# yxlao/deepSpeech

Hardware: AMD Instinct MI355X
Metric: audio-sec/sec training throughput (whole node), DS2 BiGRU (higher is better)
Workload: dtype bf16; 1 GPU; model=DeepSpeech2 2xconv(32) + 5xBiGRU-800 bidirectional + CTC, global_batch=32, seq_len=1000, parallelism=dp1, engine=hip

## Files before the change

deepspeech_amd/csrc/api.h:

```cpp
#pragma once
#include <hip/hip_runtime_api.h>
#include <stddef.h>

extern "C" {

struct DS2Fill {
  int n;
  unsigned* ptr[8];
  unsigned long long words[8];
  unsigned pattern[8];
};

hipEvent_t ds2_take_stop_event();
void ds2_arm_stop_event(hipEvent_t e);

int ds2_multi_fill(int n, void* const* ptrs, const unsigned long long* bytes, const unsigned* patterns,
                   hipStream_t st);
int ds2_multi_copy(int n, void* const* dst, const void* const* src, const unsigned long long* rows,
                   const unsigned* src_row, const unsigned* dst_row, const unsigned* src_pitch,
                   const unsigned* dst_pitch, float* sdst, const float* svals, int ns, hipStream_t st);
int ds2_wait_resident(const unsigned* word, long long timeout, hipStream_t st);
int ds2_prep_inputs(const float* x, void* y, long long n, const int* lens_in, int* lens_out, int nl,
                    hipStream_t st);
int ds2_transpose_bf16(const void* in, void* out, int R, int C, int ldi, int ldo, hipStream_t st);
// ... 214 lines not shown
                      int F, int nF, int nT, int inplace, hipStream_t st);

int ds2_seq_dropout(const void* x, void* out, const int* ctr, int T, int N, int H, unsigned seed_lo,
                    unsigned seed_hi, int site, int thr, float scale, int locked, hipStream_t st);

struct DS2Conv1WgradBn {
  const void *dz, *y1;
  const float *mean, *invstd, *gamma, *beta, *dbeta, *dgamma;
};

struct DS2Conv2DgradBn {
  const void* y1;
  const float *mean, *invstd, *gamma, *beta;
  float* part;
};

const char* ds2_conv_status_str(int rc);
size_t ds2_conv2_fwd_smem(int F1);
size_t ds2_conv2_dgrad_smem(int F2);
size_t ds2_conv2_wgrad_smem(int F1);
long long ds2_conv2_wgrad_part_floats(int grid);
long long ds2_conv1_wgrad_part_floats(int grid);
int ds2_conv1_fwd_grid(int N, int T1);
int ds2_conv1_fwd(const void* x, const void* w, const float* bias, void* y, float* part, int N, int T, int F0,
                  int T1, int F1, hipStream_t st);
int ds2_conv2_fwd(const void* x, const void* w, const float* bias, void* y, float* part, int grid, int N, int T1,
                  int F1, int T2, int F2, long long* trace, hipStream_t st);
int ds2_conv2_dgrad(const void* dy, const void* w, void* dx, int grid, int N, int T1, int F1, int T2, int F2,
                    const DS2Conv2DgradBn* bn, long long* trace, hipStream_t st);
int ds2_conv2_wgrad(const void* dy, const void* x, float* part, int grid, float* dw, int N, int T1, int F1, int T2,
                    int F2, hipStream_t st);
int ds2_conv1_wgrad(const void* dy, const void* x, float* part, int grid, float* dw, int N, int T, int F0, int T1,
                    int F1, const DS2Conv1WgradBn* bn, hipStream_t st);
int ds2_bn_cl_finalize(const float* part, int nb, double M, float eps, float* mean, float* invstd, float* run_mean,
                       float* run_var, float momentum, hipStream_t st);
int ds2_bn_cl_apply(const void* y, const float* mean, const float* invstd, const float* gamma, const float* beta,
                    void* out, int N, int T, int F, int tmaj, hipStream_t st);
int ds2_bn_cl_bwd(const void* dz, const void* y, const float* mean, const float* invstd, const float* gamma,
                  const float* beta, float* part, int nb, float* dgamma, float* dbeta, void* dy, int N, int T, int F,
                  int tmaj, int part_ready, hipStream_t st);

struct DS2Feat {
  const void* pcm;
  long long row_stride;
  int S, lead, mode, B, T_max;
  const int* lens;
  const float* offset;
  const float* gain;
  const float* basis;
  const int* mel_idx;
  const float* mel_w;
  const float* dct;
  const float* lifter;
  void* out;
  int* frames;
};

int ds2_audio_stats(const void* pcm, int in_i16, long long row_stride, int S, int B, const int* lens, float* offset,
                    float* gain, hipStream_t st);
int ds2_featurize(const DS2Feat* a, int kind, int in_i16, int out_bf16, hipStream_t st);

int ds2_resample_tile();
int ds2_resample_supported(int L, int M, int K);
int ds2_resample(const void* x, int in_i16, long long row_stride, int S, int B, const int* lens, const float* h,
                 int L, int M, int K, int in_off, int ph0, int n_out, int to_end, float* out, int* out_lens,
                 hipStream_t st);
// ... 3 lines not shown
```

deepspeech_amd/csrc/bindings.cpp:

```cpp
#include <torch/extension.h>
#include <c10/hip/HIPStream.h>
#include <hip/hip_runtime.h>

#include <algorithm>
#include <cstdint>
#include <string>
#include <utility>
#include <vector>

#include "api.h"

namespace {

using OptT = c10::optional<at::Tensor>;

hipStream_t cur_stream() { return c10::hip::getCurrentHIPStream().stream(); }

void check(int rc, const char* what) {
  TORCH_CHECK(rc == 0, "deepspeech_amd kernel launch failed in ", what, " (code ", rc, ")");
}
void check_conv(int rc, const char* what) {
  const char* why = ds2_conv_status_str(rc);
  TORCH_CHECK(rc == 0, "deepspeech_amd kernel launch failed in ", what, " (code ", rc, ")", why ? ": " : "",
              why ? why : "");
// ... 557 lines not shown
  need_bf16(x, "x"); need_bf16(w, "w"); need_bf16(y, "y");
  TORCH_CHECK(x.dim() == 4 && y.dim() == 4 && x.size(3) == 32 && y.size(3) == 32 && w.numel() == 32 * 32 * 50,
              "conv2_fwd shapes");
  TORCH_CHECK(grid > 0, "grid");
  need_f32(part, "part", grid * 64);
  check_conv(ds2_conv2_fwd(x.data_ptr(), w.data_ptr(), ptr_or_null<float>(bias, "bias"), y.data_ptr(),
                           part.data_ptr<float>(), (int)grid, (int)x.size(0), (int)x.size(1), (int)x.size(2),
                           (int)y.size(1), (int)y.size(2), trace_ptr(trace), cur_stream()), "conv2_fwd");
}

void conv2_dgrad(at::Tensor dy, at::Tensor w, at::Tensor dx, int64_t grid, OptT y1, OptT mean, OptT invstd,
                 OptT gamma, OptT beta, OptT part, OptT trace) {
  need_bf16(dy, "dy"); need_bf16(w, "w"); need_bf16(dx, "dx");
  TORCH_CHECK(dy.dim() == 4 && dx.dim() == 4 && dy.size(3) == 32 && dx.size(3) == 32 && w.numel() == 32 * 32 * 50,
              "conv2_dgrad shapes");
  TORCH_CHECK(grid > 0, "grid");
  DS2Conv2DgradBn bn{};
  const bool with_bn = y1.has_value();
  if (with_bn) {
    TORCH_CHECK(mean && invstd && gamma && beta && part, "conv2_dgrad: the BN arguments come all or none");
    need_bf16(*y1, "y1");
    TORCH_CHECK(y1->sizes() == dx.sizes(), "y1 must have dx's shape");
    need_f32(*mean, "mean", 32); need_f32(*invstd, "invstd", 32); need_f32(*gamma, "gamma", 32);
    need_f32(*beta, "beta", 32); need_f32(*part, "part", grid * 64);
    bn = DS2Conv2DgradBn{y1->data_ptr(), mean->data_ptr<float>(), invstd->data_ptr<float>(),
                         gamma->data_ptr<float>(), beta->data_ptr<float>(), part->data_ptr<float>()};
  }
  check_conv(ds2_conv2_dgrad(dy.data_ptr(), w.data_ptr(), dx.data_ptr(), (int)grid, (int)dx.size(0), (int)dx.size(1),
                             (int)dx.size(2), (int)dy.size(1), (int)dy.size(2), with_bn ? &bn : nullptr,
                             trace_ptr(trace), cur_stream()),
             "conv2_dgrad");
}

void conv2_wgrad(at::Tensor dy, at::Tensor x, at::Tensor part, at::Tensor dw, int64_t grid) {
  need_bf16(dy, "dy"); need_bf16(x, "x");
  TORCH_CHECK(grid > 0, "grid");
  need_f32(part, "part", ds2_conv2_wgrad_part_floats((int)grid));
  need_f32(dw, "dw", 32 * 32 * 50);
  check_conv(ds2_conv2_wgrad(dy.data_ptr(), x.data_ptr(), part.data_ptr<float>(), (int)grid, dw.data_ptr<float>(),
                             (int)x.size(0), (int)x.size(1), (int)x.size(2), (int)dy.size(1), (int)dy.size(2),
                             cur_stream()), "conv2_wgrad");
}

void conv1_wgrad(at::Tensor dy, at::Tensor x, at::Tensor part, at::Tensor dw, int64_t grid, OptT y1, OptT mean,
                 OptT invstd, OptT gamma, OptT beta, OptT dbeta, OptT dgamma) {
  need_bf16(dy, "dy"); need_bf16(x, "x");
  TORCH_CHECK(grid > 0, "grid");
  need_f32(part, "part", ds2_conv1_wgrad_part_floats((int)grid));
  need_f32(dw, "dw", 32 * 100);
  DS2Conv1WgradBn bn{};
  const bool with_bn = y1.has_value();
  if (with_bn) {
    TORCH_CHECK(mean && invstd && gamma && beta && dbeta && dgamma, "conv1_wgrad: the BN arguments come all or none");
    need_bf16(*y1, "y1");
    TORCH_CHECK(y1->sizes() == dy.sizes(), "y1 must have dz's shape");
    for (const OptT* t : {&mean, &invstd, &gamma, &beta, &dbeta, &dgamma}) need_f32(**t, "bn vector", 32);
    bn = DS2Conv1WgradBn{dy.data_ptr(), y1->data_ptr(), mean->data_ptr<float>(), invstd->data_ptr<float>(),
                         gamma->data_ptr<float>(), beta->data_ptr<float>(), dbeta->data_ptr<float>(),
                         dgamma->data_ptr<float>()};
  }
  check_conv(ds2_conv1_wgrad(with_bn ? nullptr : dy.data_ptr(), x.data_ptr(), part.data_ptr<float>(), (int)grid,
                             dw.data_ptr<float>(), (int)x.size(0), (int)x.size(1), (int)x.size(2), (int)dy.size(1),
                             (int)dy.size(2), with_bn ? &bn : nullptr, cur_stream()), "conv1_wgrad");
}
int64_t conv2_wgrad_part_floats(int64_t grid) { return ds2_conv2_wgrad_part_floats((int)grid); }
int64_t conv1_wgrad_part_floats(int64_t grid) { return ds2_conv1_wgrad_part_floats((int)grid); }

void bn_cl_finalize(at::Tensor part, int64_t nb, double M, double eps, at::Tensor mean, at::Tensor invstd,
                    OptT run_mean, OptT run_var, double momentum) {
  need_f32(part, "part", nb * 64);
  need_f32(mean, "mean", 32); need_f32(invstd, "invstd", 32);
  check_conv(ds2_bn_cl_finalize(part.data_ptr<float>(), (int)nb, M, (float)eps, mean.data_ptr<float>(),
                                invstd.data_ptr<float>(), ptr_or_null<float>(run_mean, "run_mean"),
                                ptr_or_null<float>(run_var, "run_var"), (float)momentum, cur_stream()),
             "bn_cl_finalize");
}

void bn_cl_apply(at::Tensor y, at::Tensor mean, at::Tensor invstd, at::Tensor gamma, at::Tensor beta, at::Tensor out,
                 bool tmaj) {
  need_bf16(y, "y"); need_bf16(out, "out");
  TORCH_CHECK(y.dim() == 4 && y.size(3) == 32 && out.numel() == y.numel(), "bn_cl_apply shapes");
  need_f32(mean, "mean", 32); need_f32(invstd, "invstd", 32); need_f32(gamma, "gamma", 32); need_f32(beta, "beta", 32);
  check_conv(ds2_bn_cl_apply(y.data_ptr(), mean.data_ptr<float>(), invstd.data_ptr<float>(), gamma.data_ptr<float>(),
                             beta.data_ptr<float>(), out.data_ptr(), (int)y.size(0), (int)y.size(1), (int)y.size(2),
                             tmaj ? 1 : 0, cur_stream()), "bn_cl_apply");
}

void bn_cl_bwd(at::Tensor dz, at::Tensor y, at::Tensor mean, at::Tensor invstd, at::Tensor gamma, at::Tensor beta,
               at::Tensor part, int64_t nb, at::Tensor dgamma, at::Tensor dbeta, at::Tensor dy, bool tmaj,
               int64_t part_ready) {
  need_bf16(dz, "dz"); need_bf16(y, "y"); need_bf16(dy, "dy");
  TORCH_CHECK(y.dim() == 4 && y.size(3) == 32 && dz.numel() == y.numel() && dy.numel() == y.numel(),
              "bn_cl_bwd shapes");
  need_f32(part, "part", nb * 64);
  need_f32(mean, "mean", 32); need_f32(invstd, "invstd", 32); need_f32(gamma, "gamma", 32); need_f32(beta, "beta", 32);
  need_f32(dgamma, "dgamma", 32); need_f32(dbeta, "dbeta", 32);
// ... 888 lines not shown
        py::arg("a_col"), py::arg("b_col"), py::arg("ws"), py::arg("cnt"), py::arg("max_grid"));
  m.def("gemm8_splits", [](int64_t K, bool fp8, int64_t S) { return ds2_gemm8_splits((int)K, fp8 ? 1 : 0, (int)S); });
  m.def("multi_fill", &multi_fill);
  m.def("col_sum", &col_sum);
  m.def("wait_resident", &wait_resident);
  m.def("fc_bias_grad", &fc_bias_grad);
  m.def("ctc_beam", &ctc_beam);
  m.def("ctc_beam_backtrack", &ctc_beam_backtrack);
  m.def("ctc_beam_lm", &ctc_beam_lm);
  m.def("ctc_beam_backtrack_lm", &ctc_beam_backtrack_lm);
  m.def("event_new", &event_new, py::arg("flags") = 0);
  m.def("arm_stop_event", &arm_stop_event);
  m.def("disarm_stop_event", &disarm_stop_event);
  m.def("event_free", &event_free);
  m.def("event_record", &event_record);
  m.def("event_wait", &event_wait);
  m.def("event_query", &event_query);
  m.def("stream_wait", &stream_wait);
  m.def("ctc_greedy", &ctc_greedy, py::arg("logits"), py::arg("lens"), py::arg("labels"), py::arg("counts"),
        py::arg("blank"), py::arg("score") = py::none());
  m.def("conv1_fwd", &conv1_fwd);
  m.def("conv1_fwd_grid", &conv1_fwd_grid);
  m.def("conv2_fwd", &conv2_fwd, py::arg("x"), py::arg("w"), py::arg("bias"), py::arg("y"), py::arg("part"),
        py::arg("grid"), py::arg("trace") = py::none());
  m.def("conv2_dgrad", &conv2_dgrad, py::arg("dy"), py::arg("w"), py::arg("dx"), py::arg("grid"),
        py::arg("y1") = py::none(), py::arg("mean") = py::none(), py::arg("invstd") = py::none(),
        py::arg("gamma") = py::none(), py::arg("beta") = py::none(), py::arg("part") = py::none(),
        py::arg("trace") = py::none());
  m.def("conv2_wgrad", &conv2_wgrad);
  m.def("conv1_wgrad", &conv1_wgrad, py::arg("dy"), py::arg("x"), py::arg("part"), py::arg("dw"), py::arg("grid"),
        py::arg("y1") = py::none(), py::arg("mean") = py::none(), py::arg("invstd") = py::none(),
        py::arg("gamma") = py::none(), py::arg("beta") = py::none(), py::arg("dbeta") = py::none(),
        py::arg("dgamma") = py::none());
  m.def("conv2_wgrad_part_floats", &conv2_wgrad_part_floats);
  m.def("conv1_wgrad_part_floats", &conv1_wgrad_part_floats);
  m.def("bn_cl_finalize", &bn_cl_finalize);
  m.def("bn_cl_apply", &bn_cl_apply);
  m.def("bn_cl_bwd", &bn_cl_bwd, py::arg("dz"), py::arg("y"), py::arg("mean"), py::arg("invstd"), py::arg("gamma"),
        py::arg("beta"), py::arg("part"), py::arg("nb"), py::arg("dgamma"), py::arg("dbeta"), py::arg("dy"),
        py::arg("tmaj"), py::arg("part_ready") = 0);
  m.def("gemm", &gemm, py::arg("A"), py::arg("B"), py::arg("C"), py::arg("bias"), py::arg("M"), py::arg("N"),
        py::arg("K"), py::arg("a_col"), py::arg("b_col"), py::arg("epi"), py::arg("alpha"), py::arg("cfg"),
        py::arg("alpha_dev") = py::none(), py::arg("Ml") = 0, py::arg("Nl") = 0, py::arg("Kl") = 0,
        py::arg("fill") = std::vector<at::Tensor>{}, py::arg("fill_pat") = std::vector<int64_t>{});
  m.def("gemm_tile", &gemm_tile);
  m.def("head_ctc", &head_ctc, py::arg("h"), py::arg("W"), py::arg("bias"), py::arg("lens"), py::arg("labels"),
        py::arg("label_lens"), py::arg("loss"), py::arg("G"), py::arg("ws"), py::arg("blank"), py::arg("zero_inf"),
        py::arg("mean") = py::none(), py::arg("counter") = py::none(), py::arg("first_bad") = py::none());
  m.def("fc_logits", &fc_logits);
  m.def("lookahead", &lookahead);
  m.def("lookahead_wgrad_parts", &lookahead_wgrad_parts);
  m.def("lookahead_wgrad", &lookahead_wgrad);
  m.def("lookahead_stream", &lookahead_stream);
  m.def("specaug_plan", &specaug_plan);
  m.def("specaug_mean", &specaug_mean);
  m.def("specaug_apply", &specaug_apply, py::arg("x"), py::arg("lens"), py::arg("plan"), py::arg("fill"),
        py::arg("out"), py::arg("nF"), py::arg("nT"), py::arg("inplace"));
  m.def("seq_dropout", &seq_dropout, py::arg("x"), py::arg("out"), py::arg("ctr"), py::arg("seed_lo"),
        py::arg("seed_hi"), py::arg("site"), py::arg("thr"), py::arg("scale"), py::arg("locked"));
  m.def("audio_stats", &audio_stats, py::arg("pcm"), py::arg("lens"), py::arg("offset"), py::arg("gain"));
  m.def("featurize", &featurize, py::arg("pcm"), py::arg("lens"), py::arg("offset"), py::arg("gain"),
        py::arg("basis"), py::arg("mel_idx"), py::arg("mel_w"), py::arg("dct"), py::arg("lifter"), py::arg("kind"),
        py::arg("lead"), py::arg("mode"), py::arg("out"), py::arg("frames"));
  m.def("resample", &resample, py::arg("pcm"), py::arg("lens"), py::arg("h"), py::arg("L"), py::arg("M"),
        py::arg("in_off"), py::arg("ph0"), py::arg("to_end"), py::arg("out"), py::arg("out_lens"));
  m.def("resample_tile", []() { return ds2_resample_tile(); });
// ... 15 lines not shown
```

deepspeech_amd/csrc/conv1.hip:

```cpp
#include "bn_math.h"
#include "conv_common.h"

using namespace ds2;

namespace {

struct Conv1Fwd {
  const bf16_t* x;
  const bf16_t* w;
  const float* bias;
  bf16_t* y;
  float* part;
  int N, T, F0, T1, F1;
};
constexpr int C1_KT = 20, C1_KF = 5;
constexpr int C1_XS = 200;
constexpr int C1_ROWS = 4;
constexpr int C1_IN = 2 * (C1_ROWS - 1) + C1_KT;

__device__ __forceinline__ void stage_rows(bf16_t* xs, const bf16_t* xu, int t0, int T, int F0) {
  constexpr int NE = C1_IN * C1_XS, K = (NE + 255) / 256;
  bf16_t v[K];
#pragma unroll
  for (int k = 0; k < K; ++k) {
    const int idx = min((int)threadIdx.x + 256 * k, NE - 1);
    const int r = idx / C1_XS, c = idx - r * C1_XS;
    v[k] = xu[(size_t)min(t0 + r, T - 1) * F0 + min(c, F0 - 1)];
  }
#pragma unroll
  for (int k = 0; k < K; ++k) {
    const int idx = (int)threadIdx.x + 256 * k;
    const int r = idx / C1_XS, c = idx - r * C1_XS;
    if (idx < NE) xs[idx] = (t0 + r < T && c < F0) ? v[k] : (bf16_t)0;
  }
}

__global__ __launch_bounds__(256) void conv1_fwd_kernel(Conv1Fwd a) {
  __shared__ __attribute__((aligned(16))) bf16_t xs[C1_IN * C1_XS];
  __shared__ __attribute__((aligned(16))) bf16_t ys[C1_ROWS][32 * MT * CC];
  __shared__ float statsh[4 * 32 * 2];
  const int tid = threadIdx.x, lane = tid & 63, w = uni(tid >> 6);
  const int hi = lane >> 5, col = lane & 31;
  const int tb = (a.T1 + C1_ROWS - 1) / C1_ROWS;
  const int n = blockIdx.x / tb, t1_0 = (blockIdx.x - n * tb) * C1_ROWS;
  stage_rows(xs, a.x + (size_t)n * a.T * a.F0, 2 * t1_0, a.T, a.F0);
  bf16x8 bfr[10];
#pragma unroll
  for (int s = 0; s < 10; ++s) {
    const int kt = 2 * s + hi;
    bf16x8 v;
#pragma unroll
    for (int j = 0; j < 8; ++j) v[j] = j < C1_KF ? (short)a.w[(col * C1_KT + kt) * C1_KF + j] : (short)0;
    bfr[s] = v;
  }
  const float bco = a.bias ? a.bias[col] : 0.f;
  __syncthreads();
  float ssum = 0.f, ssq = 0.f;
  const int t1 = t1_0 + w;
  if (t1 < a.T1) {
    f32x16 acc[MT];
#pragma unroll
    for (int m = 0; m < MT; ++m) acc[m] = (f32x16){};
#pragma unroll
    for (int s = 0; s < 10; ++s) {
      const int r = 2 * w + 2 * s + hi;
#pragma unroll
      for (int m = 0; m < MT; ++m) {
// ... 3 lines not shown
        acc[m] = mfma32(av, bfr[s], acc[m]);
      }
    }
    bf16_t* yl = ys[w];
#pragma unroll
    for (int m = 0; m < MT; ++m)
#pragma unroll
      for (int r = 0; r < 16; ++r) {
        const int f1 = 32 * m + (r & 3) + 8 * (r >> 2) + 4 * hi;
        if (f1 < a.F1) {
          const bf16_t b = f2bf(acc[m][r] + bco);
          yl[f1 * CC + col] = b;
          const float vb = bf2f(b);
          ssum += vb;
          ssq += vb * vb;
        }
      }
    copy_row(a.y + ((size_t)n * a.T1 + t1) * a.F1 * CC, yl, a.F1 * 4, lane, 64);
  }
  channel_sums(ssum, ssq, statsh, w, a.part);
}

struct Conv1Wgrad {
  const bf16_t* dy;
  const bf16_t* x;
  float* part;
  int N, T, F0, T1, F1;
  DS2Conv1WgradBn bn;
  float M;
};
constexpr int C1W_XP = 88;
constexpr int C1W_DY = C1_ROWS * 80 * 64;
constexpr int C1W_XD = C1_IN * 8 * C1W_XP * 2;
constexpr int C1W_RED = 4 * 5 * 4 * 64 * 16;
constexpr int C1W_RAW = C1_IN * C1_XS * 2;
constexpr int C1W_SMEM = (C1W_DY + C1W_XD + C1W_RAW) > C1W_RED ? (C1W_DY + C1W_XD + C1W_RAW) : C1W_RED;

__global__ __launch_bounds__(256) void conv1_wgrad_kernel(Conv1Wgrad a) {
  extern __shared__ __attribute__((aligned(16))) unsigned char smem[];
  const int tid = threadIdx.x, lane = tid & 63, w = uni(tid >> 6);
  const int hi = lane >> 5, col = lane & 31;
  unsigned char* dys = smem;
  bf16_t* xd = (bf16_t*)(smem + C1W_DY);
  bf16_t* raw = (bf16_t*)(smem + C1W_DY + C1W_XD);
  const int tb = (a.T1 + C1_ROWS - 1) / C1_ROWS;
  const int ntiles = a.N * tb;
  const unsigned lofs = tr_lane_ofs(lane);
  const int bkt = col >> 3, bkf = col & 7;

  const bool bn = a.bn.dz != nullptr;
  const bf16_t *bdz = (const bf16_t*)a.bn.dz, *by1 = (const bf16_t*)a.bn.y1;
  float bmu[8], bis[8], bg[8], bbt[8], bmdb[8], bmdg[8];
  if (bn) {
#pragma unroll
    for (int j = 0; j < 8; ++j) {
      const int c = (tid & 3) * 8 + j;
      bmu[j] = a.bn.mean[c]; bis[j] = a.bn.invstd[c]; bg[j] = a.bn.gamma[c]; bbt[j] = a.bn.beta[c];
      bmdb[j] = a.bn.dbeta[c] / a.M; bmdg[j] = a.bn.dgamma[c] / a.M;
    }
  }
  f32x16 acc[5];
#pragma unroll
  for (int i = 0; i < 5; ++i) acc[i] = (f32x16){};
  for (int tile = blockIdx.x; tile < ntiles; tile += gridDim.x) {
    const int n = tile / tb, t1_0 = (tile - n * tb) * C1_ROWS;
    __syncthreads();
    for (int ch = tid; ch < C1_ROWS * 80 * 4; ch += 256) {
      const int r = ch / 320, rem = ch - r * 320, pos = rem >> 2, c4 = rem & 3;
      const int t1 = t1_0 + r;
      i32x4 v = (i32x4){0, 0, 0, 0};
      if (pos < a.F1 && t1 < a.T1) {
        const size_t off = (((size_t)n * a.T1 + t1) * a.F1 + pos) * CC + c4 * 8;
        if (bn) {
          const bf16x8 y = *(const bf16x8*)(by1 + off), d = *(const bf16x8*)(bdz + off);
          bf16x8 o;
#pragma unroll
          for (int j = 0; j < 8; ++j) {
            const float xh = bn_xhat(bf2f((bf16_t)y[j]), bmu[j], bis[j]);
            const float dd = bn_masked(xh, bg[j], bbt[j], bf2f((bf16_t)d[j]));
            o[j] = (short)f2bf(bn_bwd_value(bg[j] * bis[j], dd, xh, bmdb[j], bmdg[j]));
          }
          v = __builtin_bit_cast(i32x4, o);
        } else {
          v = *(const i32x4*)(a.dy + off);
        }
      }
      *(i32x4*)(dys + ch * 16) = v;
    }
    stage_rows(raw, a.x + (size_t)n * a.T * a.F0, 2 * t1_0, a.T, a.F0);
    __syncthreads();
    for (int ch = tid; ch < C1_IN * 8 * 10; ch += 256) {
      const int kf = ch & 7, q = ch >> 3, r = q / 10, p0 = (q - r * 10) * 8;
      bf16x8 v;
#pragma unroll
      for (int j = 0; j < 8; ++j) v[j] = (short)raw[r * C1_XS + min(2 * (p0 + j) + kf, C1_XS - 1)];
      *(bf16x8*)(xd + (r * 8 + kf) * C1W_XP + p0) = v;
    }
    __syncthreads();
    const int t1 = t1_0 + w;
    if (t1 < a.T1) {
#pragma unroll
      for (int kk = 0; kk < 5; ++kk) {
        const unsigned k0 = (unsigned)(16 * kk);
        const bf16x8 av = tr_frag(dys + (w * 80 + k0) * 64 + lofs);
#pragma unroll
        for (int nt = 0; nt < 5; ++nt) {
          const int r = 2 * w + 4 * nt + bkt;
          const bf16x8 bv = *(const bf16x8*)(xd + (r * 8 + bkf) * C1W_XP + k0 + 8 * hi);
          acc[nt] = mfma32(av, bv, acc[nt]);
        }
      }
    }
  }
  __syncthreads();
  f32x4* red = (f32x4*)smem;
#pragma unroll
  for (int nt = 0; nt < 5; ++nt)
#pragma unroll
    for (int r4 = 0; r4 < 4; ++r4) red[((w * 5 + nt) * 4 + r4) * 64 + lane] = acc4(acc[nt], r4);
  __syncthreads();
  f32x4* out = (f32x4*)(a.part + (size_t)blockIdx.x * 5 * 1024);
  for (int e = tid; e < 5 * 4 * 64; e += 256) {
    f32x4 v = red[e];
    for (int wv = 1; wv < 4; ++wv) v += red[wv * 5 * 4 * 64 + e];
    out[e] = v;
  }
}

bool conv1_geometry(int T, int F0, int T1, int F1, int F1max) {
  return F1 <= F1max && F1 == (F0 - 5) / 2 + 1 && T1 == (T - 20) / 2 + 1 && T1 >= 1;
}

}

extern "C" {

long long ds2_conv1_wgrad_part_floats(int grid) { return (long long)grid * 5 * 1024; }
int ds2_conv1_fwd_grid(int N, int T1) { return N * ((T1 + C1_ROWS - 1) / C1_ROWS); }

int ds2_conv1_fwd(const void* x, const void* w, const float* bias, void* y, float* part, int N, int T, int F0,
                  int T1, int F1, hipStream_t st) {
  if (!conv1_geometry(T, F0, T1, F1, 96)) return CONV1_FWD_GEOMETRY;
  Conv1Fwd a{(const bf16_t*)x, (const bf16_t*)w, bias, (bf16_t*)y, part, N, T, F0, T1, F1};
  hipLaunchKernelGGL(conv1_fwd_kernel, dim3(ds2_conv1_fwd_grid(N, T1)), dim3(256), 0, st, a);
  return (int)hipGetLastError();
}

int ds2_conv1_wgrad(const void* dy, const void* x, float* part, int grid, float* dw, int N, int T, int F0, int T1,
                    int F1, const DS2Conv1WgradBn* bn, hipStream_t st) {
  if (!conv1_geometry(T, F0, T1, F1, 80)) return CONV1_WGRAD_GEOMETRY;
  if ((dy == nullptr) == (bn == nullptr)) return CONV1_WGRAD_DY_XOR_BN;
  DS2_HIP_CHECK((hipError_t)set_smem(conv1_wgrad_kernel, C1W_SMEM));
  Conv1Wgrad a{(const bf16_t*)dy, (const bf16_t*)x, part, N, T, F0, T1, F1, bn ? *bn : DS2Conv1WgradBn{},
               (float)((double)N * T1 * F1)};
  hipLaunchKernelGGL(conv1_wgrad_kernel, dim3(grid), dim3(256), C1W_SMEM, st, a);
  hipLaunchKernelGGL(wgrad_reduce_kernel<1>, dim3(5 * 1024 / 256), dim3(256), 0, st, part, grid, 5 * 1024, dw);
  return (int)hipGetLastError();
}

}
```

deepspeech_amd/csrc/conv2.hip:

```cpp
#include "bn_math.h"
#include "conv_common.h"

using namespace ds2;

namespace {

constexpr int PR = 80;

template <int KPW, int S0, typename Idx>
__device__ __forceinline__ void gather_wfrag(bf16x8 (&bfr)[KPW], const unsigned short* wl, int hh, int hi, int col,
                                             Idx idx) {
#pragma unroll
  for (int i = 0; i < KPW; ++i) {
    const int s = S0 + i;
    if ((s & 1) != hh) continue;
    const int kt = s / 10, kf = (s % 10) >> 1;
#pragma unroll
    for (int j = 0; j < 8; ++j) bfr[i][j] = (short)wl[idx(8 * hi + j, col, kt, kf)];
  }
}

struct Conv2Fwd {
  const bf16_t* x;
  const bf16_t* w;
// ... 355 lines not shown
    if (tile + (int)gridDim.x < ntiles) issue(tile + gridDim.x, (it & 1) ? buf0 : buf1);
    const unsigned char* xs = cur + dyBytes;
#pragma unroll
    for (int kk = 0; kk < 5; ++kk) {
      const unsigned k0 = (unsigned)(16 * kk) * 64u;
      const bf16x8 av = tr_frag(cur + k0 + lofs);
#pragma unroll
      for (int i = 0; i < C2W_PPW; ++i) {
        if (i < npairs) {
          const int P = w + C2W_WAVES * i;
          const int kt = P / 5, kf = P - 5 * (P / 5);
          acc[i] = mfma32(av, tr_frag(xs + (unsigned)(kt * a.F1 + kf) * 64u + k0 + lofs), acc[i]);
        }
      }
    }
  }
  f32x4* out = (f32x4*)(a.part + (size_t)blockIdx.x * C2W_PAIRS * 1024);
#pragma unroll
  for (int i = 0; i < C2W_PPW; ++i) {
    if (i < npairs) {
      const int P = w + C2W_WAVES * i;
#pragma unroll
      for (int r4 = 0; r4 < 4; ++r4) out[(P * 4 + r4) * 64 + lane] = acc4(acc[i], r4);
    }
  }
}

int shape_ok(int T1, int F1, int T2, int F2) {
  if (F1 < 5 || F1 > 80 || F2 != F1 - 4) return CONV2_F_RANGE;
  if (T1 < 10 || T2 != (T1 - 10) / 2 + 1) return CONV2_T_RANGE;
  return 0;
}

}

extern "C" {

const char* ds2_conv_status_str(int rc) {
  switch (rc) {
#define X(name, value, meaning) \
  case value: return meaning;
    DS2_CONV_STATUS(X)
#undef X
  }
  return nullptr;
}

size_t ds2_conv2_fwd_smem(int) { return (size_t)C2F_SMEM; }
size_t ds2_conv2_dgrad_smem(int) { return (size_t)C2D_SMEM; }
size_t ds2_conv2_wgrad_smem(int F1) { return (size_t)2 * (80 * 64 + (9 * F1 + 84) * 64); }
long long ds2_conv2_wgrad_part_floats(int grid) { return (long long)grid * C2W_PAIRS * 1024; }

int ds2_conv2_fwd(const void* x, const void* w, const float* bias, void* y, float* part, int grid, int N, int T1,
                  int F1, int T2, int F2, long long* trace, hipStream_t st) {
  if (int e = shape_ok(T1, F1, T2, F2)) return e;
  const size_t smem = ds2_conv2_fwd_smem(F1);
  DS2_HIP_CHECK((hipError_t)set_smem(conv2_fwd_kernel, smem));
  Conv2Fwd a{(const bf16_t*)x, (const bf16_t*)w, bias, (bf16_t*)y, part, N, T1, F1, T2, F2, trace};
  hipLaunchKernelGGL(conv2_fwd_kernel, dim3(grid), dim3(256), smem, st, a);
  return (int)hipGetLastError();
}

int ds2_conv2_dgrad(const void* dy, const void* w, void* dx, int grid, int N, int T1, int F1, int T2, int F2,
                    const DS2Conv2DgradBn* bn, long long* trace, hipStream_t st) {
  if (int e = shape_ok(T1, F1, T2, F2)) return e;
  if (F1 <= 64) return CONV2_DGRAD_NARROW;
  const size_t smem = ds2_conv2_dgrad_smem(F2);
  DS2_HIP_CHECK((hipError_t)set_smem(conv2_dgrad_kernel, smem));
  Conv2Dgrad a{(const bf16_t*)dy, (const bf16_t*)w, (bf16_t*)dx, N, T1, F1, T2, F2,
               bn ? *bn : DS2Conv2DgradBn{}, trace};
  hipLaunchKernelGGL(conv2_dgrad_kernel, dim3(grid), dim3(256), smem, st, a);
  return (int)hipGetLastError();
}

int ds2_conv2_wgrad(const void* dy, const void* x, float* part, int grid, float* dw, int N, int T1, int F1, int T2,
                    int F2, hipStream_t st) {
  if (int e = shape_ok(T1, F1, T2, F2)) return e;
  const size_t smem = ds2_conv2_wgrad_smem(F1);
  DS2_HIP_CHECK((hipError_t)set_smem(conv2_wgrad_kernel, smem));
  Conv2Wgrad a{(const bf16_t*)dy, (const bf16_t*)x, part, N, T1, F1, T2, F2};
  hipLaunchKernelGGL(conv2_wgrad_kernel, dim3(grid), dim3(512), smem, st, a);
  hipLaunchKernelGGL(wgrad_reduce_kernel<0>, dim3(C2W_PAIRS * 1024 / 256), dim3(256), 0, st, part, grid,
                     C2W_PAIRS * 1024, dw);
  return (int)hipGetLastError();
}

}
```

deepspeech_amd/csrc/conv_common.h:

```cpp
#pragma once
#include "common.h"

#define DS2_CONV_STATUS(X)                                                                                 \
  X(CONV2_F_RANGE, -40, "conv2 needs 5 <= F1 <= 80 and F2 = F1 - 4 (LDS row planes, staging capacity)")    \
  X(CONV2_T_RANGE, -41, "conv2 needs T1 >= 10 and T2 = (T1 - 10) / 2 + 1")                                  \
  X(CONV2_DGRAD_NARROW, -42, "conv2_dgrad needs F1 > 64: it stores positions 0..63 of a row unchecked")     \
  X(CONV1_WGRAD_GEOMETRY, -43, "conv1_wgrad needs F1 = (F0 - 5) / 2 + 1 <= 80, T1 = (T - 20) / 2 + 1 >= 1") \
  X(CONV1_WGRAD_DY_XOR_BN, -44, "conv1_wgrad takes dy or the BatchNorm backward's inputs, exactly one")     \
  X(BN_CL_BWD_WIDE, -45, "bn_cl_bwd needs F <= 96")                                                         \
  X(BN_CL_BWD_TMAJ_READY, -46, "bn_cl_bwd: part_ready excludes tmaj (that path transposes in its reduce)")  \
  X(CONV1_FWD_GEOMETRY, -47, "conv1_fwd needs F1 = (F0 - 5) / 2 + 1 <= 96, T1 = (T - 20) / 2 + 1 >= 1")     \
  X(BN_CL_APPLY_WIDE, -48, "bn_cl_apply needs F <= 96 (one LDS row of the time-major transpose)")

namespace ds2 {

enum ConvStatus : int {
#define X(name, value, meaning) name = value,
  DS2_CONV_STATUS(X)
#undef X
};

typedef __attribute__((ext_vector_type(16))) float f32x16;
typedef __attribute__((ext_vector_type(4))) short s16x4;
typedef __attribute__((address_space(3))) void lds_void_t;
// ... 48 lines not shown
__device__ __forceinline__ void c2_stamp(long long* tr, int it, int k) {
  if (tr != nullptr && blockIdx.x < 8 && threadIdx.x == 0 && it < 16)
    tr[((int)blockIdx.x * 16 + it) * C2_TRACE + k] = __builtin_amdgcn_s_memrealtime();
}

__device__ __forceinline__ void copy_row(bf16_t* dst, const void* lds_row, int chunks, int first, int step) {
  for (int q = first; q < chunks; q += step) ((i32x4*)dst)[q] = ((const i32x4*)lds_row)[q];
}

__device__ __forceinline__ void channel_sums(float s, float q, float* sh, int w, float* part) {
  const int tid = threadIdx.x, lane = tid & 63;
  s += __shfl_xor(s, 32, 64);
  q += __shfl_xor(q, 32, 64);
  __syncthreads();
  if (lane < 32) {
    sh[(w * 32 + lane) * 2 + 0] = s;
    sh[(w * 32 + lane) * 2 + 1] = q;
  }
  __syncthreads();
  if (tid < 64) part[(size_t)blockIdx.x * 64 + tid] = sh[tid] + sh[64 + tid] + sh[128 + tid] + sh[192 + tid];
}

template <typename K>
int set_smem(K kernel, size_t bytes) {
  return (int)hipFuncSetAttribute(reinterpret_cast<const void*>(kernel), hipFuncAttributeMaxDynamicSharedMemorySize,
                                  (int)bytes);
}

}

namespace {

template <int KIND>
__global__ __launch_bounds__(256) void wgrad_reduce_kernel(const float* __restrict__ part, int nb, int E,
                                                           float* __restrict__ dw) {
  using namespace ds2;
  __shared__ f32x4 sh[4][64];
  const int tid = threadIdx.x, g = tid >> 6, l = tid & 63;
  const int e4 = blockIdx.x * 64 + l, E4 = E >> 2;
  const f32x4* p4 = (const f32x4*)part;
  f32x4 s0 = {}, s1 = {};
  int b = g;
  for (; b + 4 < nb; b += 8) {
    s0 += p4[(size_t)b * E4 + e4];
    s1 += p4[(size_t)(b + 4) * E4 + e4];
  }
  if (b < nb) s0 += p4[(size_t)b * E4 + e4];
  sh[g][l] = s0 + s1;
  __syncthreads();
  if (g != 0) return;
  const f32x4 v = sh[0][l] + sh[1][l] + sh[2][l] + sh[3][l];
#pragma unroll
  for (int j = 0; j < 4; ++j) {
    const int e = e4 * 4 + j;
    const int P = e >> 10, rem = e & 1023, r4 = rem >> 8, ln = (rem >> 2) & 63;
    const int row = (rem & 3) + 8 * r4 + 4 * (ln >> 5), c = ln & 31;
    if (KIND == 0) {
      const int kt = P / 5, kf = P % 5;
      dw[((row * CC + c) * C2_KT + kt) * C2_KF + kf] = v[j];
    } else {
      const int kt = 4 * P + (c >> 3), kf = c & 7;
      if (kf < 5) dw[(row * 20 + kt) * 5 + kf] = v[j];
    }
  }
}

}
```

deepspeech_amd/ops/frontend.py:

```python
from __future__ import annotations

import os

import torch
import torch.nn.functional as F

from . import _ext
from .optim import arena_of, emit_grad
from ..utils import trace as TR

_HEAD_SIDE = True

BN_EPS = 1e-3
BN_MOMENTUM = 0.01



_C1W_BPC = 1

_CONV_WSIDE = os.environ.get("DS2_CONV_WSIDE", "0") == "1"
_conv_streams = {}



def _conv_side_stream(dev, w):
    a = arena_of(w)
    if not _CONV_WSIDE or dev.type != "cuda" or (a is not None and getattr(a, "_ready_cbs", None)):
        return None
    idx = dev.index if dev.index is not None else torch.cuda.current_device()
    s = _conv_streams.get(idx)
    if s is None:
        s = _conv_streams[idx] = torch.cuda.Stream(device=torch.device("cuda", idx))
    return s

def bn_eval_stats(block, eps: float):
    if getattr(block, "bn", "fused") == "moments_ema":
        m, v = block.ema_moments()
        return m.float().contiguous(), torch.rsqrt(v.float() + eps).contiguous()
    return block.running_mean.float().contiguous(), torch.rsqrt(block.running_var.float() + eps).contiguous()


def bn_track(block, mean: torch.Tensor, invstd: torch.Tensor, eps: float) -> None:
    if getattr(block, "bn", "fused") == "moments_ema":
        block.ema_update(mean, invstd.pow(-2) - eps)


def _stat_buffers(block, dev):
    if getattr(block, "bn", "fused") == "moments_ema":
        return torch.zeros(block.bn_gamma.numel(), device=dev), torch.ones(block.bn_gamma.numel(), device=dev)
    return block.running_mean, block.running_var

# ... 205 lines not shown
        dev = x.device
        f32 = dict(device=dev, dtype=torch.float32)
        dout = dout.to(torch.bfloat16).contiguous()
        N, T2, F2, _ = y2.shape
        T1 = y1.shape[1]
        grid = max(1, min(N * T2, ctx.ncu))
        nb2 = max(1, min(N * T2, 1024))
        part = torch.empty(max(2 * ctx.ncu, nb2) * 64, **f32)
        with TR.phase(TR.bn(2, True)):
            (dg2, ipg2), (db2, ipb2) = _grad_buffer(g2), _grad_buffer(be2)
            dy2 = torch.empty_like(y2)
            C_.bn_cl_bwd(dout, y2, mean2, inv2, g2f, be2f, part, nb2, dg2, db2, dy2, True)
        side = _conv_side_stream(dev, w2)
        main = torch.cuda.current_stream(dev) if side is not None else None
        with TR.phase(TR.conv(2, True)):
            wpart = torch.empty(int(C_.conv2_wgrad_part_floats(grid)), **f32)
            dw2, ip2 = _grad_buffer(w2)
            if side is not None:
                from .rnn import _stream_wait
                _stream_wait(side, main)
                with torch.cuda.stream(side):
                    C_.conv2_wgrad(dy2, z1, wpart, dw2, grid)
            dz1 = torch.empty_like(y1)
            dgrid = max(1, min(N * ((T1 + 1) // 2), 2 * ctx.ncu))
            C_.conv2_dgrad(dy2, w2_16, dz1, dgrid, y1, mean1, inv1, g1f, be1f, part)
        gg2, gb2, gbias2 = _deliver(g2, dg2, ipg2), _deliver(be2, db2, ipb2), _zero_grad_of(b2)
        with TR.phase(TR.bn(1, True)):
            (dg1, ipg1), (db1, ipb1) = _grad_buffer(g1), _grad_buffer(be1)
            C_.bn_cl_bwd(dz1, y1, mean1, inv1, g1f, be1f, part, dgrid, dg1, db1, dz1, False, part_ready=2)
        with TR.phase(TR.conv(1, True)):
            g1grid = max(1, min(N * ((T1 + 3) // 4), _C1W_BPC * ctx.ncu))
            wpart1 = torch.empty(int(C_.conv1_wgrad_part_floats(g1grid)), **f32)
            dw1, ip1 = _grad_buffer(w1)
            C_.conv1_wgrad(dz1, x, wpart1, dw1, g1grid, y1, mean1, inv1, g1f, be1f, db1, dg1)
            if side is not None:
                _stream_wait(main, side)
                gw2 = _deliver(w2, dw2, ip2)
            else:
                C_.conv2_wgrad(dy2, z1, wpart, dw2, grid)
                gw2 = _deliver(w2, dw2, ip2)
            gw1 = _deliver(w1, dw1, ip1)
        gg1, gb1, gbias1 = _deliver(g1, dg1, ipg1), _deliver(be1, db1, ipb1), _zero_grad_of(b1)
        return None, gw1, gbias1, gg1, gb1, gw2, gbias2, gg2, gb2, None


CL_F1_FORWARD = (9, 80)
CL_F1_TRAINING = (65, 80)


def cl_supported(model, feats: torch.Tensor) -> bool:
    if model.num_filters != 32 or feats.dim() != 3:
        return False
    F1 = (feats.shape[2] - 5) // 2 + 1
    lo, hi = CL_F1_TRAINING if model.conv1.training else CL_F1_FORWARD
    return lo <= F1 <= hi and feats.shape[1] >= 38


def frontend_hip(model, feats: torch.Tensor) -> torch.Tensor:
    if cl_supported(model, feats) and os.environ.get("DS2_CONV", "hip") == "hip":
        c1, c2 = model.conv1, model.conv2
        return FrontendCL.apply(feats, c1.weight, c1.bias, c1.bn_gamma, c1.bn_beta,
                                c2.weight, c2.bias, c2.bn_gamma, c2.bn_beta, model)
    x = feats.unsqueeze(1)
    x = conv_block_hip(model.conv1, x, 0, 1)
    if getattr(model, "capture", False):
        model.act_taps["conv1"] = x.detach()
    x = conv_block_hip(model.conv2, x, 1, 2)
    if getattr(model, "capture", False):
        model.act_taps["conv2"] = x.detach()
    return x

# ... 54 lines not shown
```

Before: 41920 audio-sec/sec.

## Prefetch conv1 wgrad tiles into registers and merge the two wgrad reductions

Rewrites the conv1 weight-gradient kernel so that the next tile's global loads are issued into registers while the current tile is computed. It specialises the kernel on BN with a template and keeps the BN constants in LDS, reduces accumulators in chunks to cut LDS use, and doubles blocks per CU. It also merges the conv1 and conv2 partial-sum reductions into one launch and unrolls the reduction loop deeper. The aim is to hide load latency and save a launch in the conv backward, at the cost of extra register pressure and a smaller share of the step, which is dominated by the GRUs.

```diff
diff --git a/deepspeech_amd/csrc/api.h b/deepspeech_amd/csrc/api.h
--- a/deepspeech_amd/csrc/api.h
+++ b/deepspeech_amd/csrc/api.h
@@ -270,6 +270,8 @@
                     int F2, hipStream_t st);
 int ds2_conv1_wgrad(const void* dy, const void* x, float* part, int grid, float* dw, int N, int T, int F0, int T1,
                     int F1, const DS2Conv1WgradBn* bn, hipStream_t st);
+int ds2_wgrad_reduce2(const float* part2, int grid2, float* dw2, const float* part1, int grid1, float* dw1,
+                      hipStream_t st);
 int ds2_bn_cl_finalize(const float* part, int nb, double M, float eps, float* mean, float* invstd, float* run_mean,
                        float* run_var, float momentum, hipStream_t st);
 int ds2_bn_cl_apply(const void* y, const float* mean, const float* invstd, const float* gamma, const float* beta,
diff --git a/deepspeech_amd/csrc/bindings.cpp b/deepspeech_amd/csrc/bindings.cpp
--- a/deepspeech_amd/csrc/bindings.cpp
+++ b/deepspeech_amd/csrc/bindings.cpp
@@ -613,22 +613,23 @@
              "conv2_dgrad");
 }
 
-void conv2_wgrad(at::Tensor dy, at::Tensor x, at::Tensor part, at::Tensor dw, int64_t grid) {
+void conv2_wgrad(at::Tensor dy, at::Tensor x, at::Tensor part, OptT dw, int64_t grid) {
   need_bf16(dy, "dy"); need_bf16(x, "x");
   TORCH_CHECK(grid > 0, "grid");
   need_f32(part, "part", ds2_conv2_wgrad_part_floats((int)grid));
-  need_f32(dw, "dw", 32 * 32 * 50);
-  check_conv(ds2_conv2_wgrad(dy.data_ptr(), x.data_ptr(), part.data_ptr<float>(), (int)grid, dw.data_ptr<float>(),
+  if (dw) need_f32(*dw, "dw", 32 * 32 * 50);
+  check_conv(ds2_conv2_wgrad(dy.data_ptr(), x.data_ptr(), part.data_ptr<float>(), (int)grid,
+                             dw ? dw->data_ptr<float>() : nullptr,
                              (int)x.size(0), (int)x.size(1), (int)x.size(2), (int)dy.size(1), (int)dy.size(2),
                              cur_stream()), "conv2_wgrad");
 }
 
-void conv1_wgrad(at::Tensor dy, at::Tensor x, at::Tensor part, at::Tensor dw, int64_t grid, OptT y1, OptT mean,
+void conv1_wgrad(at::Tensor dy, at::Tensor x, at::Tensor part, OptT dw, int64_t grid, OptT y1, OptT mean,
                  OptT invstd, OptT gamma, OptT beta, OptT dbeta, OptT dgamma) {
   need_bf16(dy, "dy"); need_bf16(x, "x");
   TORCH_CHECK(grid > 0, "grid");
   need_f32(part, "part", ds2_conv1_wgrad_part_floats((int)grid));
-  need_f32(dw, "dw", 32 * 100);
+  if (dw) need_f32(*dw, "dw", 32 * 100);
   DS2Conv1WgradBn bn{};
   const bool with_bn = y1.has_value();
   if (with_bn) {
@@ -641,8 +642,18 @@
                          dgamma->data_ptr<float>()};
   }
   check_conv(ds2_conv1_wgrad(with_bn ? nullptr : dy.data_ptr(), x.data_ptr(), part.data_ptr<float>(), (int)grid,
-                             dw.data_ptr<float>(), (int)x.size(0), (int)x.size(1), (int)x.size(2), (int)dy.size(1),
-                             (int)dy.size(2), with_bn ? &bn : nullptr, cur_stream()), "conv1_wgrad");
+                             dw ? dw->data_ptr<float>() : nullptr, (int)x.size(0), (int)x.size(1), (int)x.size(2),
+                             (int)dy.size(1), (int)dy.size(2), with_bn ? &bn : nullptr, cur_stream()), "conv1_wgrad");
+}
+
+void wgrad_reduce2(at::Tensor part2, int64_t grid2, at::Tensor dw2, at::Tensor part1, int64_t grid1, at::Tensor dw1) {
+  TORCH_CHECK(grid1 > 0 && grid2 > 0, "grid");
+  need_f32(part2, "part2", ds2_conv2_wgrad_part_floats((int)grid2));
+  need_f32(part1, "part1", ds2_conv1_wgrad_part_floats((int)grid1));
+  need_f32(dw2, "dw2", 32 * 32 * 50);
+  need_f32(dw1, "dw1", 32 * 100);
+  check_conv(ds2_wgrad_reduce2(part2.data_ptr<float>(), (int)grid2, dw2.data_ptr<float>(), part1.data_ptr<float>(),
+                               (int)grid1, dw1.data_ptr<float>(), cur_stream()), "wgrad_reduce2");
 }
 int64_t conv2_wgrad_part_floats(int64_t grid) { return ds2_conv2_wgrad_part_floats((int)grid); }
 int64_t conv1_wgrad_part_floats(int64_t grid) { return ds2_conv1_wgrad_part_floats((int)grid); }
@@ -1597,6 +1608,7 @@
         py::arg("y1") = py::none(), py::arg("mean") = py::none(), py::arg("invstd") = py::none(),
         py::arg("gamma") = py::none(), py::arg("beta") = py::none(), py::arg("dbeta") = py::none(),
         py::arg("dgamma") = py::none());
+  m.def("wgrad_reduce2", &wgrad_reduce2);
   m.def("conv2_wgrad_part_floats", &conv2_wgrad_part_floats);
   m.def("conv1_wgrad_part_floats", &conv1_wgrad_part_floats);
   m.def("bn_cl_finalize", &bn_cl_finalize);
diff --git a/deepspeech_amd/csrc/conv1.hip b/deepspeech_amd/csrc/conv1.hip
--- a/deepspeech_amd/csrc/conv1.hip
+++ b/deepspeech_amd/csrc/conv1.hip
@@ -18,21 +18,27 @@
 constexpr int C1_ROWS = 4;
 constexpr int C1_IN = 2 * (C1_ROWS - 1) + C1_KT;
 
-__device__ __forceinline__ void stage_rows(bf16_t* xs, const bf16_t* xu, int t0, int T, int F0) {
-  constexpr int NE = C1_IN * C1_XS, K = (NE + 255) / 256;
-  bf16_t v[K];
-#pragma unroll
-  for (int k = 0; k < K; ++k) {
-    const int idx = min((int)threadIdx.x + 256 * k, NE - 1);
+constexpr int C1_NE = C1_IN * C1_XS, C1_K = (C1_NE + 255) / 256;
+__device__ __forceinline__ void load_rows(bf16_t (&v)[C1_K], const bf16_t* xu, int t0, int T, int F0, int tid) {
+#pragma unroll
+  for (int k = 0; k < C1_K; ++k) {
+    const int idx = min(tid + 256 * k, C1_NE - 1);
     const int r = idx / C1_XS, c = idx - r * C1_XS;
     v[k] = xu[(size_t)min(t0 + r, T - 1) * F0 + min(c, F0 - 1)];
   }
-#pragma unroll
-  for (int k = 0; k < K; ++k) {
-    const int idx = (int)threadIdx.x + 256 * k;
+}
+__device__ __forceinline__ void store_rows(bf16_t* xs, const bf16_t (&v)[C1_K], int t0, int T, int F0, int tid) {
+#pragma unroll
+  for (int k = 0; k < C1_K; ++k) {
+    const int idx = tid + 256 * k;
     const int r = idx / C1_XS, c = idx - r * C1_XS;
-    if (idx < NE) xs[idx] = (t0 + r < T && c < F0) ? v[k] : (bf16_t)0;
-  }
+    if (idx < C1_NE) xs[idx] = (t0 + r < T && c < F0) ? v[k] : (bf16_t)0;
+  }
+}
+__device__ __forceinline__ void stage_rows(bf16_t* xs, const bf16_t* xu, int t0, int T, int F0) {
+  bf16_t v[C1_K];
+  load_rows(v, xu, t0, T, F0, (int)threadIdx.x);
+  store_rows(xs, v, t0, T, F0, (int)threadIdx.x);
 }
 
 __global__ __launch_bounds__(256) void conv1_fwd_kernel(Conv1Fwd a) {
@@ -102,63 +108,108 @@
 constexpr int C1W_XP = 88;
 constexpr int C1W_DY = C1_ROWS * 80 * 64;
 constexpr int C1W_XD = C1_IN * 8 * C1W_XP * 2;
-constexpr int C1W_RED = 4 * 5 * 4 * 64 * 16;
 constexpr int C1W_RAW = C1_IN * C1_XS * 2;
-constexpr int C1W_SMEM = (C1W_DY + C1W_XD + C1W_RAW) > C1W_RED ? (C1W_DY + C1W_XD + C1W_RAW) : C1W_RED;
-
-__global__ __launch_bounds__(256) void conv1_wgrad_kernel(Conv1Wgrad a) {
+constexpr int C1W_CST = 6 * CC * 4;
+constexpr int C1W_NTP = 3;
+constexpr int C1W_RED = 4 * C1W_NTP * 4 * 64 * 16;
+constexpr int C1W_TILE = C1W_DY + C1W_XD + C1W_RAW + C1W_CST;
+constexpr int C1W_SMEM = C1W_TILE > C1W_RED ? C1W_TILE : C1W_RED;
+constexpr int C1W_CH = C1_ROWS * 80 * 4 / 256;
+
+template <bool BN>
+struct C1wRegs {
+  i32x4 d[C1W_CH];
+  i32x4 y[BN ? C1W_CH : 1];
+  bf16_t x[C1_K];
+};
+
+template <bool BN>
+__device__ __forceinline__ void c1w_issue(C1wRegs<BN>& p, const Conv1Wgrad& a, int n, int t1_0, int tid) {
+  const bf16_t* pd = BN ? (const bf16_t*)a.bn.dz : a.dy;
+  const bf16_t* py = (const bf16_t*)a.bn.y1;
+#pragma unroll
+  for (int k = 0; k < C1W_CH; ++k) {
+    const int ch = tid + 256 * k;
+    const int r = ch / 320, rem = ch - r * 320, pos = rem >> 2, c4 = rem & 3;
+    const size_t off = (((size_t)n * a.T1 + min(t1_0 + r, a.T1 - 1)) * a.F1 + min(pos, a.F1 - 1)) * CC + c4 * 8;
+    p.d[k] = *(const i32x4*)(pd + off);
+    if (BN) p.y[k] = *(const i32x4*)(py + off);
+  }
+  load_rows(p.x, a.x + (size_t)n * a.T * a.F0, 2 * t1_0, a.T, a.F0, tid);
+}
+
+template <bool BN>
+__device__ __forceinline__ void c1w_land(const C1wRegs<BN>& p, const Conv1Wgrad& a, int t1_0, int tid,
+                                         unsigned char* dys, bf16_t* raw, const float* cst) {
+  float bmu[8], bis[8], bg[8], bbt[8], bmdb[8], bmdg[8];
+  if (BN) {
+    const float* c = cst + (tid & 3) * 8;
+#pragma unroll
+    for (int j = 0; j < 8; ++j) {
+      bmu[j] = c[j]; bis[j] = c[CC + j]; bg[j] = c[2 * CC + j]; bbt[j] = c[3 * CC + j];
+      bmdb[j] = c[4 * CC + j]; bmdg[j] = c[5 * CC + j];
+    }
+  }
+#pragma unroll
+  for (int k = 0; k < C1W_CH; ++k) {
+    const int ch = tid + 256 * k;
+    const int r = ch / 320, rem = ch - r * 320, pos = rem >> 2;
+    i32x4 v = p.d[k];
+    if (BN) {
+      const bf16x8 y = __builtin_bit_cast(bf16x8, p.y[k]), d = __builtin_bit_cast(bf16x8, p.d[k]);
+      bf16x8 o;
+#pragma unroll
+      for (int j = 0; j < 8; ++j) {
+        const float xh = bn_xhat(bf2f((bf16_t)y[j]), bmu[j], bis[j]);
+        const float dd = bn_masked(xh, bg[j], bbt[j], bf2f((bf16_t)d[j]));
+        o[j] = (short)f2bf(bn_bwd_value(bg[j] * bis[j], dd, xh, bmdb[j], bmdg[j]));
+      }
+      v = __builtin_bit_cast(i32x4, o);
+    }
+    const bool live = pos < a.F1 && t1_0 + r < a.T1;
+    *(i32x4*)(dys + ch * 16) = live ? v : (i32x4){0, 0, 0, 0};
+  }
+  store_rows(raw, p.x, 2 * t1_0, a.T, a.F0, tid);
+}
+
+template <bool BN>
+__global__ __launch_bounds__(256) __attribute__((amdgpu_waves_per_eu(2, 2))) void conv1_wgrad_kernel(Conv1Wgrad a) {
   extern __shared__ __attribute__((aligned(16))) unsigned char smem[];
   const int tid = threadIdx.x, lane = tid & 63, w = uni(tid >> 6);
   const int hi = lane >> 5, col = lane & 31;
   unsigned char* dys = smem;
   bf16_t* xd = (bf16_t*)(smem + C1W_DY);
   bf16_t* raw = (bf16_t*)(smem + C1W_DY + C1W_XD);
+  float* cst = (float*)(smem + C1W_DY + C1W_XD + C1W_RAW);
   const int tb = (a.T1 + C1_ROWS - 1) / C1_ROWS;
   const int ntiles = a.N * tb;
   const unsigned lofs = tr_lane_ofs(lane);
   const int bkt = col >> 3, bkf = col & 7;
 
-  const bool bn = a.bn.dz != nullptr;
-  const bf16_t *bdz = (const bf16_t*)a.bn.dz, *by1 = (const bf16_t*)a.bn.y1;
-  float bmu[8], bis[8], bg[8], bbt[8], bmdb[8], bmdg[8];
-  if (bn) {
-#pragma unroll
-    for (int j = 0; j < 8; ++j) {
-      const int c = (tid & 3) * 8 + j;
-      bmu[j] = a.bn.mean[c]; bis[j] = a.bn.invstd[c]; bg[j] = a.bn.gamma[c]; bbt[j] = a.bn.beta[c];
-      bmdb[j] = a.bn.dbeta[c] / a.M; bmdg[j] = a.bn.dgamma[c] / a.M;
-    }
+  float c6[6];
+  if (BN && tid < CC) {
+    c6[0] = a.bn.mean[tid]; c6[1] = a.bn.invstd[tid]; c6[2] = a.bn.gamma[tid]; c6[3] = a.bn.beta[tid];
+    c6[4] = a.bn.dbeta[tid]; c6[5] = a.bn.dgamma[tid];
+  }
+  C1wRegs<BN> p;
+  int tile = blockIdx.x;
+  if (tile < ntiles) c1w_issue<BN>(p, a, tile / tb, (tile % tb) * C1_ROWS, tid);
+  if (BN && tid < CC) {
+#pragma unroll
+    for (int i = 0; i < 6; ++i) cst[i * CC + tid] = i < 4 ? c6[i] : c6[i] / a.M;
   }
   f32x16 acc[5];
 #pragma unroll
   for (int i = 0; i < 5; ++i) acc[i] = (f32x16){};
-  for (int tile = blockIdx.x; tile < ntiles; tile += gridDim.x) {
-    const int n = tile / tb, t1_0 = (tile - n * tb) * C1_ROWS;
-    __syncthreads();
-    for (int ch = tid; ch < C1_ROWS * 80 * 4; ch += 256) {
-      const int r = ch / 320, rem = ch - r * 320, pos = rem >> 2, c4 = rem & 3;
-      const int t1 = t1_0 + r;
-      i32x4 v = (i32x4){0, 0, 0, 0};
-      if (pos < a.F1 && t1 < a.T1) {
-        const size_t off = (((size_t)n * a.T1 + t1) * a.F1 + pos) * CC + c4 * 8;
-        if (bn) {
-          const bf16x8 y = *(const bf16x8*)(by1 + off), d = *(const bf16x8*)(bdz + off);
-          bf16x8 o;
-#pragma unroll
-          for (int j = 0; j < 8; ++j) {
-            const float xh = bn_xhat(bf2f((bf16_t)y[j]), bmu[j], bis[j]);
-            const float dd = bn_masked(xh, bg[j], bbt[j], bf2f((bf16_t)d[j]));
-            o[j] = (short)f2bf(bn_bwd_value(bg[j] * bis[j], dd, xh, bmdb[j], bmdg[j]));
-          }
-          v = __builtin_bit_cast(i32x4, o);
-        } else {
-          v = *(const i32x4*)(a.dy + off);
-        }
-      }
-      *(i32x4*)(dys + ch * 16) = v;
-    }
-    stage_rows(raw, a.x + (size_t)n * a.T * a.F0, 2 * t1_0, a.T, a.F0);
-    __syncthreads();
+  for (; tile < ntiles; tile += gridDim.x) {
+    const int t1_0 = (tile % tb) * C1_ROWS;
+    int ltid = tid;
+    asm volatile("" : "+v"(ltid));
+    lds_barrier();
+    c1w_land<BN>(p, a, t1_0, ltid, dys, raw, cst);
+    lds_barrier();
+    const int next = tile + (int)gridDim.x;
+    if (next < ntiles) c1w_issue<BN>(p, a, next / tb, (next % tb) * C1_ROWS, ltid);
     for (int ch = tid; ch < C1_IN * 8 * 10; ch += 256) {
       const int kf = ch & 7, q = ch >> 3, r = q / 10, p0 = (q - r * 10) * 8;
       bf16x8 v;
@@ -166,7 +217,7 @@
       for (int j = 0; j < 8; ++j) v[j] = (short)raw[r * C1_XS + min(2 * (p0 + j) + kf, C1_XS - 1)];
       *(bf16x8*)(xd + (r * 8 + kf) * C1W_XP + p0) = v;
     }
-    __syncthreads();
+    lds_barrier();
     const int t1 = t1_0 + w;
     if (t1 < a.T1) {
 #pragma unroll
@@ -182,18 +233,23 @@
       }
     }
   }
-  __syncthreads();
   f32x4* red = (f32x4*)smem;
-#pragma unroll
-  for (int nt = 0; nt < 5; ++nt)
-#pragma unroll
-    for (int r4 = 0; r4 < 4; ++r4) red[((w * 5 + nt) * 4 + r4) * 64 + lane] = acc4(acc[nt], r4);
-  __syncthreads();
   f32x4* out = (f32x4*)(a.part + (size_t)blockIdx.x * 5 * 1024);
-  for (int e = tid; e < 5 * 4 * 64; e += 256) {
-    f32x4 v = red[e];
-    for (int wv = 1; wv < 4; ++wv) v += red[wv * 5 * 4 * 64 + e];
-    out[e] = v;
+#pragma unroll
+  for (int nt0 = 0; nt0 < 5; nt0 += C1W_NTP) {
+    constexpr int WS = C1W_NTP * 4 * 64;
+    const int cnt = (5 - nt0 < C1W_NTP ? 5 - nt0 : C1W_NTP) * 4 * 64;
+    __syncthreads();
+#pragma unroll
+    for (int nt = nt0; nt < 5 && nt < nt0 + C1W_NTP; ++nt)
+#pragma unroll
+      for (int r4 = 0; r4 < 4; ++r4) red[w * WS + ((nt - nt0) * 4 + r4) * 64 + lane] = acc4(acc[nt], r4);
+    __syncthreads();
+    for (int e = tid; e < cnt; e += 256) {
+      f32x4 v = red[e];
+      for (int wv = 1; wv < 4; ++wv) v += red[wv * WS + e];
+      out[nt0 * 4 * 64 + e] = v;
+    }
   }
 }
 
@@ -220,11 +276,13 @@
                     int F1, const DS2Conv1WgradBn* bn, hipStream_t st) {
   if (!conv1_geometry(T, F0, T1, F1, 80)) return CONV1_WGRAD_GEOMETRY;
   if ((dy == nullptr) == (bn == nullptr)) return CONV1_WGRAD_DY_XOR_BN;
-  DS2_HIP_CHECK((hipError_t)set_smem(conv1_wgrad_kernel, C1W_SMEM));
+  const auto kernel = bn ? conv1_wgrad_kernel<true> : conv1_wgrad_kernel<false>;
+  DS2_HIP_CHECK((hipError_t)set_smem(kernel, C1W_SMEM));
   Conv1Wgrad a{(const bf16_t*)dy, (const bf16_t*)x, part, N, T, F0, T1, F1, bn ? *bn : DS2Conv1WgradBn{},
                (float)((double)N * T1 * F1)};
-  hipLaunchKernelGGL(conv1_wgrad_kernel, dim3(grid), dim3(256), C1W_SMEM, st, a);
-  hipLaunchKernelGGL(wgrad_reduce_kernel<1>, dim3(5 * 1024 / 256), dim3(256), 0, st, part, grid, 5 * 1024, dw);
+  hipLaunchKernelGGL(kernel, dim3(grid), dim3(256), C1W_SMEM, st, a);
+  if (dw != nullptr)
+    hipLaunchKernelGGL(wgrad_reduce_kernel<1>, dim3(5 * 1024 / 256), dim3(256), 0, st, part, grid, 5 * 1024, dw);
   return (int)hipGetLastError();
 }
 
diff --git a/deepspeech_amd/csrc/conv2.hip b/deepspeech_amd/csrc/conv2.hip
--- a/deepspeech_amd/csrc/conv2.hip
+++ b/deepspeech_amd/csrc/conv2.hip
@@ -411,6 +411,16 @@
   return 0;
 }
 
+__global__ __launch_bounds__(256) void wgrad_reduce2_kernel(const float* __restrict__ part2, int nb2,
+                                                            float* __restrict__ dw2, const float* __restrict__ part1,
+                                                            int nb1, float* __restrict__ dw1) {
+  constexpr int B2 = C2W_PAIRS * 1024 / 256;
+  if ((int)blockIdx.x < B2)
+    wgrad_reduce_block<0>(part2, nb2, C2W_PAIRS * 1024, dw2, (int)blockIdx.x);
+  else
+    wgrad_reduce_block<1>(part1, nb1, 5 * 1024, dw1, (int)blockIdx.x - B2);
+}
+
 }
 
 extern "C" {
@@ -459,9 +469,17 @@
   DS2_HIP_CHECK((hipError_t)set_smem(conv2_wgrad_kernel, smem));
   Conv2Wgrad a{(const bf16_t*)dy, (const bf16_t*)x, part, N, T1, F1, T2, F2};
   hipLaunchKernelGGL(conv2_wgrad_kernel, dim3(grid), dim3(512), smem, st, a);
-  hipLaunchKernelGGL(wgrad_reduce_kernel<0>, dim3(C2W_PAIRS * 1024 / 256), dim3(256), 0, st, part, grid,
-                     C2W_PAIRS * 1024, dw);
+  if (dw != nullptr)
+    hipLaunchKernelGGL(wgrad_reduce_kernel<0>, dim3(C2W_PAIRS * 1024 / 256), dim3(256), 0, st, part, grid,
+                       C2W_PAIRS * 1024, dw);
   return (int)hipGetLastError();
 }
 
-}
+int ds2_wgrad_reduce2(const float* part2, int grid2, float* dw2, const float* part1, int grid1, float* dw1,
+                      hipStream_t st) {
+  hipLaunchKernelGGL(wgrad_reduce2_kernel, dim3((C2W_PAIRS + 5) * 1024 / 256), dim3(256), 0, st, part2, grid2, dw2,
+                     part1, grid1, dw1);
+  return (int)hipGetLastError();
+}
+
+}
diff --git a/deepspeech_amd/csrc/conv_common.h b/deepspeech_amd/csrc/conv_common.h
--- a/deepspeech_amd/csrc/conv_common.h
+++ b/deepspeech_amd/csrc/conv_common.h
@@ -104,15 +104,25 @@
 namespace {
 
 template <int KIND>
-__global__ __launch_bounds__(256) void wgrad_reduce_kernel(const float* __restrict__ part, int nb, int E,
-                                                           float* __restrict__ dw) {
+__device__ __forceinline__ void wgrad_reduce_block(const float* __restrict__ part, int nb, int E,
+                                                   float* __restrict__ dw, int block) {
   using namespace ds2;
   __shared__ f32x4 sh[4][64];
   const int tid = threadIdx.x, g = tid >> 6, l = tid & 63;
-  const int e4 = blockIdx.x * 64 + l, E4 = E >> 2;
+  const int e4 = block * 64 + l, E4 = E >> 2;
   const f32x4* p4 = (const f32x4*)part;
   f32x4 s0 = {}, s1 = {};
   int b = g;
+  for (; b + 28 < nb; b += 32) {
+    f32x4 v[8];
+#pragma unroll
+    for (int k = 0; k < 8; ++k) v[k] = p4[(size_t)(b + 4 * k) * E4 + e4];
+#pragma unroll
+    for (int k = 0; k < 4; ++k) {
+      s0 += v[2 * k];
+      s1 += v[2 * k + 1];
+    }
+  }
   for (; b + 4 < nb; b += 8) {
     s0 += p4[(size_t)b * E4 + e4];
     s1 += p4[(size_t)(b + 4) * E4 + e4];
@@ -137,4 +147,10 @@
   }
 }
 
+template <int KIND>
+__global__ __launch_bounds__(256) void wgrad_reduce_kernel(const float* __restrict__ part, int nb, int E,
+                                                           float* __restrict__ dw) {
+  wgrad_reduce_block<KIND>(part, nb, E, dw, (int)blockIdx.x);
 }
+
+}
diff --git a/deepspeech_amd/ops/frontend.py b/deepspeech_amd/ops/frontend.py
--- a/deepspeech_amd/ops/frontend.py
+++ b/deepspeech_amd/ops/frontend.py
@@ -16,7 +16,8 @@
 
 
 
-_C1W_BPC = 1
+_C1W_BPC = 2
+_WGRAD_JOINT = True
 
 _CONV_WSIDE = os.environ.get("DS2_CONV_WSIDE", "0") == "1"
 _conv_streams = {}
@@ -288,11 +289,17 @@
             g1grid = max(1, min(N * ((T1 + 3) // 4), _C1W_BPC * ctx.ncu))
             wpart1 = torch.empty(int(C_.conv1_wgrad_part_floats(g1grid)), **f32)
             dw1, ip1 = _grad_buffer(w1)
-            C_.conv1_wgrad(dz1, x, wpart1, dw1, g1grid, y1, mean1, inv1, g1f, be1f, db1, dg1)
             if side is not None:
+                C_.conv1_wgrad(dz1, x, wpart1, dw1, g1grid, y1, mean1, inv1, g1f, be1f, db1, dg1)
                 _stream_wait(main, side)
                 gw2 = _deliver(w2, dw2, ip2)
+            elif _WGRAD_JOINT:
+                C_.conv1_wgrad(dz1, x, wpart1, None, g1grid, y1, mean1, inv1, g1f, be1f, db1, dg1)
+                C_.conv2_wgrad(dy2, z1, wpart, None, grid)
+                C_.wgrad_reduce2(wpart, grid, dw2, wpart1, g1grid, dw1)
+                gw2 = _deliver(w2, dw2, ip2)
             else:
+                C_.conv1_wgrad(dz1, x, wpart1, dw1, g1grid, y1, mean1, inv1, g1f, be1f, db1, dg1)
                 C_.conv2_wgrad(dy2, z1, wpart, dw2, grid)
                 gw2 = _deliver(w2, dw2, ip2)
             gw1 = _deliver(w1, dw1, ip1)
```

Result: no change. 42210 audio-sec/sec (median of 6 runs) (+0.7%).
